# Francesco215/autoregressive_diffusion

Hardware: AMD Instinct MI355X
Metric: denoiser-step frames/sec at 1/2/4/8 MI355X; 64-frame Lunar-Lander seq (higher is better)
Workload: dtype bf16; 1 GPU; Lunar-Lander 64-frame seq, gym EDM2 UNet 46.2M (gym_train.py:37-47), 8 seq/GPU (gym_train.py:55 micro_batch_size), step = EDM2Loss fwd + bwd + grad all-reduce + [grad-norm clip +] AdamW + 2 EMA profiles, 3:1 mix of 3-D/2-D steps; global_batch=8, seq_len=64, parallelism=dp1, hip_graph=False

## Files before the change

### autoregressive_diffusion_amd/_lib.py

```python
import ctypes as C
import os

import torch

_HERE = os.path.dirname(os.path.abspath(__file__))
LIB_PATH = os.path.join(_HERE, os.environ.get("ONIRIS_LIB_NAME", "liboniris_hip.so"))

if not os.path.exists(LIB_PATH):
    raise ImportError(f"{LIB_PATH} not found: build the HIP extension first (make -j8 at the repo root); "
                      "there is no CPU/PyTorch fallback for the denoiser kernels")

lib = C.CDLL(LIB_PATH)

c_void_p, c_int, c_float, c_int32, c_int64, c_size_t = C.c_void_p, C.c_int, C.c_float, C.c_int32, C.c_int64, C.c_size_t


class WeightDesc(C.Structure):
    _fields_ = [("w", c_void_p), ("grad", c_void_p), ("wf", c_void_p), ("wb", c_void_p), ("dwp", c_void_p), ("dws", c_void_p),
                ("cout", c_int32), ("cin", c_int32), ("taps", c_int32), ("kt", c_int32),
                ("CoutP", c_int32), ("CinP", c_int32), ("CoutPb", c_int32), ("CinPb", c_int32),
                ("row_start", c_int32), ("perm3", c_int32), ("gain", c_float), ("nsplit_cap", c_int32),
                ("nsplit", c_void_p), ("tile_start", c_int32), ("pad_", c_int32)]


# ... 42 lines not shown
                ("dout", c_void_p), ("delta", c_void_p), ("dq", c_void_p), ("dk", c_void_p), ("dv", c_void_p),
                ("BH", c_int32), ("Lq", c_int32), ("Lk", c_int32), ("D", c_int32), ("mask_mode", c_int32), ("P", c_int32),
                ("T", c_int32), ("q_frame_off", c_int32), ("scale", c_float), ("pad_", c_int32)]


EPI_NONE, EPI_EMB_SILU, EPI_MPSUM, EPI_ACT_BWD = 0, 1, 2, 3

_SIGS = {
    "oniris_last_error": (C.c_char_p, []),
    "oniris_abi_version": (c_int, []),
    "oniris_struct_sizes": (c_int, [c_void_p]),
    "oniris_profile_arm": (c_int, [c_void_p, c_void_p]),
    "oniris_profile_disarm": (c_int, []),
    "oniris_set_cu_reserve": (c_int, [c_int]),
    "oniris_set_ew_nt_bytes": (c_int64, [c_int64]),
    "oniris_frame_attn_bwd": (c_int, [c_void_p, c_void_p]),
    "oniris_frame_attn_qkv_fwd": (c_int, [c_void_p, c_void_p, c_void_p, c_int64, c_int, c_int, c_void_p]),
    "oniris_frame_attn_qkv_bwd": (c_int, [c_void_p, c_void_p, c_void_p, c_void_p, c_void_p, c_int64, c_int, c_int, c_void_p]),
    "oniris_conv_f32": (c_int, [c_void_p, c_void_p, c_void_p, c_int64, c_int, c_int, c_int, c_int, c_int, c_void_p]),
    "oniris_wgrad_f32": (c_int, [c_void_p, c_void_p, c_void_p, c_int64, c_int, c_int, c_int, c_int, c_int, c_void_p]),
    "oniris_attn_f32_fwd": (c_int, [c_void_p, c_void_p]),
    "oniris_attn_f32_bwd": (c_int, [c_void_p, c_void_p]),
    "oniris_census": (c_int, [c_int]),
    "oniris_census_read": (c_int64, [C.c_char_p, c_int64]),
    "oniris_train_mask": (c_int, [c_int, c_int, c_void_p, c_void_p, C.POINTER(c_int)]),
    "oniris_infer_mask": (c_int, [c_int, c_int, c_void_p, c_void_p, C.POINTER(c_int)]),
    "oniris_mask_transpose": (c_int, [c_int, c_int, c_void_p, c_void_p, c_void_p, c_void_p]),
    "oniris_attn_schedule": (c_int, [c_int, c_int, c_void_p, c_int, c_void_p, c_int]),
    "oniris_weight_prep": (c_int, [c_void_p, c_int, c_int, c_int, c_int, c_void_p]),
    "oniris_weight_bwd": (c_int, [c_void_p, c_int, c_int, c_void_p]),
# ... 202 lines not shown
```

### autoregressive_diffusion_amd/csrc/common.h

```cpp
#pragma once
#include <hip/hip_runtime.h>
#include <hip/hip_ext.h>
#include <stdint.h>
#include <stdio.h>
#include <string.h>

typedef __bf16 bf16;
typedef __attribute__((ext_vector_type(8))) __bf16 bf16x8;
typedef __attribute__((ext_vector_type(4))) __bf16 bf16x4;
typedef __attribute__((ext_vector_type(2))) __bf16 bf16x2;
typedef __attribute__((ext_vector_type(4))) short s16x4;
typedef __attribute__((ext_vector_type(16))) float f32x16;
typedef __attribute__((ext_vector_type(4))) float f32x4;
typedef __attribute__((ext_vector_type(4))) unsigned int u32x4;

#define ONIRIS_OK 0
#define ONIRIS_EINVAL (-1)
#define ONIRIS_ELAUNCH (-2)
#define ONIRIS_EUNSUPPORTED (-3)

void oniris_set_error(const char* fmt, ...);

#define ONIRIS_CHECK_ARG(cond, ...)                \
  do {                                             \
// ... 38 lines not shown
  oniris_launch_tagged(nullptr, kern, grid, block, stream, args...);
}

long long oniris_ew_nt_bytes(void);
template <bool NT, typename V>
__device__ __forceinline__ V ldv(const V* p) {
  if constexpr (NT) return __builtin_nontemporal_load(p);
  else return *p;
}
template <bool NT, typename V>
__device__ __forceinline__ void stv(V* p, V v) {
  if constexpr (NT) __builtin_nontemporal_store(v, p);
  else *p = v;
}

extern int oniris_cu_reserve;
int oniris_persistent_wgs(void);

static inline int cdiv(int a, int b) { return (a + b - 1) / b; }
static inline int roundup(int a, int b) { return cdiv(a, b) * b; }

#ifdef __HIPCC__
__device__ __forceinline__ float bf2f(bf16 v) { return (float)v; }
__device__ __forceinline__ bf16 f2bf(float v) { return (bf16)v; }

__device__ __forceinline__ f32x16 mfma32(bf16x8 a, bf16x8 b, f32x16 c) {
  return __builtin_amdgcn_mfma_f32_32x32x16_bf16(a, b, c, 0, 0, 0);
}
__device__ __forceinline__ float sigmoid_fast(float z) {
  return __builtin_amdgcn_rcpf(1.f + __builtin_amdgcn_exp2f(-1.4426950408889634f * z));
}
__device__ __forceinline__ float act_adjoint_da(float da, float xo) {
  const float sg = sigmoid_fast(xo);
  const float one_m = 1.f - sg;
  const float u = __builtin_fmaf(one_m, xo, 1.f);
  float g = sg * u;
  g = g * da;
  return g * (1.0f / 0.596f);
}
__device__ __forceinline__ float act_adjoint_dxo(float g, float dxo_scale, float dxo) { return __builtin_fmaf(dxo_scale, dxo, g); }
__device__ __forceinline__ float act_adjoint_out(float g, float w, bool has_add, float add) {
  return has_add ? __builtin_fmaf(w, g, add) : g * w;
}
__device__ __forceinline__ int mfma_row(int r, int lane) { return (r & 3) + 8 * (r >> 2) + 4 * (lane >> 5); }

__device__ __forceinline__ float wave_sum(float v) {
#pragma unroll
  for (int o = 32; o > 0; o >>= 1) v += __shfl_xor(v, o);
  return v;
}
__device__ __forceinline__ float wave_max(float v) {
#pragma unroll
  for (int o = 32; o > 0; o >>= 1) v = fmaxf(v, __shfl_xor(v, o));
  return v;
}

__device__ __forceinline__ float block_sum(float v, float* red) {
  v = wave_sum(v);
  const int w = threadIdx.x >> 6, nw = blockDim.x >> 6;
  __syncthreads();
  if ((threadIdx.x & 63) == 0) red[w] = v;
  __syncthreads();
  float t = 0.f;
  for (int i = 0; i < nw; ++i) t += red[i];
  return t;
}
#endif
```

### autoregressive_diffusion_amd/csrc/elementwise.hip

```cpp
#include <cstdlib>
#include "common.h"
#include "../../include/oniris.h"

#define SILU_SCALE (1.0f / 0.596f)

__device__ __forceinline__ float silu_f(float z) { return z * sigmoid_fast(z); }
__device__ __forceinline__ float dsilu_f(float z) {
  const float sg = sigmoid_fast(z);
  return sg * (1.f + z * (1.f - sg));
}

template <bool NORM, bool NT>
__global__ __launch_bounds__(256) void act_fwd_kernel(const bf16* __restrict__ x, const bf16* __restrict__ skip,
                                                      bf16* __restrict__ xo, bf16* __restrict__ a,
                                                      float* __restrict__ sden, long long npix, int C1, int C2, float w1,
                                                      float w2, int rs, int Ho, int Wo) {
  const int C = C1 + C2, G = C >> 3;
  const long long gid = (long long)blockIdx.x * 256 + threadIdx.x;
  const long long pix = gid / G;
  const int cg = (int)(gid % G);
  const bool ok = pix < npix;
  float v[8];
#pragma unroll
  for (int i = 0; i < 8; ++i) v[i] = 0.f;
// ... 148 lines not shown
  const int C = C1 + C2;
  ONIRIS_CHECK_ARG(da && xo && dx && npix > 0 && C1 > 0 && C1 % 8 == 0 && C2 >= 0 && C2 % 8 == 0 && (C2 == 0 || dskip),
                   "act_bwd: bad arguments");
  ONIRIS_CHECK_ARG(!norm || ((C / 8) <= 64 && ((C / 8) & (C / 8 - 1)) == 0 && sden), "act_bwd: pixel norm needs C/8 = 2^k <= 64");
  const long long nthr = npix * (C / 8);
  const dim3 grid((unsigned)((nthr + 255) / 256));
  const bool nt = (long long)npix * C * 2 >= oniris_ew_nt_bytes();
#define ACT_BWD_LAUNCH(NORM_, NT_) ONIRIS_KLAUNCH((act_bwd_kernel<NORM_, NT_>), grid, dim3(256), 0, stream, (const bf16*)da, (const bf16*)dxo, (const bf16*)xo, sden, (bf16*)dx, (bf16*)dskip, (const bf16*)dadd, (long long)npix, C1, C2, w1, w2, dxo_scale)
  if (norm) { if (nt) ACT_BWD_LAUNCH(true, true); else ACT_BWD_LAUNCH(true, false); }
  else { if (nt) ACT_BWD_LAUNCH(false, true); else ACT_BWD_LAUNCH(false, false); }
#undef ACT_BWD_LAUNCH
  ONIRIS_LAUNCH_CHECK();
  return ONIRIS_OK;
}

template <bool NT>
__global__ __launch_bounds__(256) void emb_silu_bwd_kernel(const bf16* __restrict__ du, const bf16* __restrict__ y,
                                                           const float* __restrict__ c, bf16* __restrict__ dy,
                                                           float* __restrict__ dc, int P, int C, int pix_per_block,
                                                           int c_pitch) {
  __shared__ float acc[512];
  const int n = blockIdx.x, G = C >> 3;
  const int cg = threadIdx.x % G, pl = threadIdx.x / G, npl = 256 / G;
  for (int i = threadIdx.x; i < C; i += 256) acc[i] = 0.f;
  __syncthreads();
  float cv[8], part[8];
#pragma unroll
  for (int i = 0; i < 8; ++i) { cv[i] = 0.f; part[i] = 0.f; }
  if (pl < npl) {
    const float4 c0 = *(const float4*)(c + (size_t)n * c_pitch + cg * 8), c1 = *(const float4*)(c + (size_t)n * c_pitch + cg * 8 + 4);
    cv[0] = c0.x; cv[1] = c0.y; cv[2] = c0.z; cv[3] = c0.w; cv[4] = c1.x; cv[5] = c1.y; cv[6] = c1.z; cv[7] = c1.w;
    const int p0 = blockIdx.y * pix_per_block;
    const int p1 = min(P, p0 + pix_per_block);
    for (int p = p0 + pl; p < p1; p += npl) {
      const size_t off = ((size_t)n * P + p) * C + cg * 8;
      const bf16x8 duv = ldv<NT>((const bf16x8*)(du + off)), yv = ldv<NT>((const bf16x8*)(y + off));
      bf16x8 o;
#pragma unroll
      for (int i = 0; i < 8; ++i) {
        const float yy = bf2f(yv[i]);
        const float dz = bf2f(duv[i]) * dsilu_f(yy * cv[i]) * SILU_SCALE;
        o[i] = f2bf(dz * cv[i]);
        part[i] += dz * yy;
      }
      stv<NT>((bf16x8*)(dy + off), o);
    }
  }
  if ((G & (G - 1)) == 0) {
#pragma unroll
    for (int i = 0; i < 8; ++i)
      for (int o = G; o < 64; o <<= 1) part[i] += __shfl_xor(part[i], o);
    for (int q = 0; q < 256 / 64; ++q) {
      if ((int)(threadIdx.x >> 6) == q && (int)(threadIdx.x & 63) < G)
#pragma unroll
        for (int i = 0; i < 8; ++i) acc[cg * 8 + i] += part[i];
      __syncthreads();
    }
  } else {
    for (int q = 0; q < npl; ++q) {
      if (pl == q)
#pragma unroll
        for (int i = 0; i < 8; ++i) acc[cg * 8 + i] += part[i];
      __syncthreads();
    }
  }
  for (int i = threadIdx.x; i < C; i += 256) atomicAdd(dc + (size_t)n * C + i, acc[i]);
}

__global__ void zero_f32_kernel(float* __restrict__ p, size_t n) {
  const size_t i = (size_t)blockIdx.x * blockDim.x + threadIdx.x;
  if (i < n) p[i] = 0.f;
}

extern "C" int oniris_emb_silu_bwd(const void* du, const void* y, const float* c, void* dy, float* dc, int N, int P,
                                   int C, int c_pitch, int dc_is_zero, oniris_stream_t stream_) {
  hipStream_t stream = (hipStream_t)stream_;
  ONIRIS_CHECK_ARG(du && y && c && dy && dc && N > 0 && P > 0 && C > 0 && C % 8 == 0 && C <= 512,
                   "emb_silu_bwd: bad arguments (C %% 8 == 0, C <= 512)");
  int slices = 1;
  const int npl = 256 / (C / 8) > 0 ? 256 / (C / 8) : 1;
  static int tgt = -1;
  if (tgt < 0) { const char* e = getenv("ONIRIS_EMB_SILU_BLOCKS"); tgt = e ? atoi(e) : 1024; }
  while (slices < 2 && P / (slices * 2) >= npl * 4 && (long long)N * slices < tgt) slices *= 2;
  const int ppb = cdiv(P, slices);
  const size_t ndc = (size_t)N * C;
  if (!dc_is_zero) ONIRIS_KLAUNCH(zero_f32_kernel, dim3((unsigned)((ndc + 255) / 256)), dim3(256), 0, stream, dc, ndc);
  const int cp = c_pitch > 0 ? c_pitch : C;
  ONIRIS_CHECK_ARG(cp >= C && cp % 4 == 0, "emb_silu_bwd: c_pitch must be a multiple of 4 and >= C");
  if ((long long)N * P * C * 2 >= oniris_ew_nt_bytes())
    ONIRIS_KLAUNCH(emb_silu_bwd_kernel<true>, dim3(N, slices), dim3(256), 0, stream, (const bf16*)du, (const bf16*)y, c,
                       (bf16*)dy, dc, P, C, ppb, cp);
  else
    ONIRIS_KLAUNCH(emb_silu_bwd_kernel<false>, dim3(N, slices), dim3(256), 0, stream, (const bf16*)du, (const bf16*)y, c,
                       (bf16*)dy, dc, P, C, ppb, cp);
  ONIRIS_LAUNCH_CHECK();
  return ONIRIS_OK;
}

template <bool NT>
__global__ void mpsum_bwd_kernel(const bf16* __restrict__ g, const bf16* __restrict__ out, bf16* __restrict__ dres,
                                 bf16* __restrict__ dv, size_t n8, float ta, float tb, float clip) {
  for (size_t i = (size_t)blockIdx.x * blockDim.x + threadIdx.x; i < n8; i += (size_t)gridDim.x * blockDim.x) {
    const bf16x8 gv = ldv<NT>((const bf16x8*)(g + i * 8));
    bf16x8 a, b;
    if (clip > 0.f) {
      const bf16x8 ov = ldv<NT>((const bf16x8*)(out + i * 8));
#pragma unroll
      for (int k = 0; k < 8; ++k) {
        const float gg = (fabsf(bf2f(ov[k])) < clip) ? bf2f(gv[k]) : 0.f;
// ... 707 lines not shown
```

### autoregressive_diffusion_amd/csrc/misc.cpp

```cpp
#include <cstdlib>
#include <stdarg.h>
#include <stdio.h>
#include <string.h>
#include <algorithm>
#include <map>
#include <mutex>
#include <string>
#include <vector>
#include <cxxabi.h>
#include <dlfcn.h>
#include <hip/hip_runtime.h>
#include "common.h"
#include "../../include/oniris.h"

static thread_local char g_err[512] = "";

void oniris_set_error(const char* fmt, ...) {
  va_list ap;
  va_start(ap, fmt);
  vsnprintf(g_err, sizeof(g_err), fmt, ap);
  va_end(ap);
}

extern "C" const char* oniris_last_error(void) { return g_err; }
// ... 15 lines not shown
static long long g_ew_nt_bytes = -1;
long long oniris_ew_nt_bytes(void) {
  if (g_ew_nt_bytes < 0) {
    const char* e = getenv("ONIRIS_EW_NT_MB");
    const long long mb = e ? atoll(e) : 96;
    g_ew_nt_bytes = mb <= 0 ? (1LL << 62) : mb * (1LL << 20);
  }
  return g_ew_nt_bytes;
}
extern "C" long long oniris_set_ew_nt_bytes(long long bytes) {
  const long long old = oniris_ew_nt_bytes();
  g_ew_nt_bytes = bytes < 0 ? (1LL << 62) : bytes;
  return old;
}

int oniris_census_on = 0;
static std::mutex g_census_mu;
static std::map<std::pair<const void*, std::string>, long long> g_census;
void oniris_census_note(const void* h, const char* tag) {
  std::lock_guard<std::mutex> lock(g_census_mu);
  ++g_census[std::make_pair(h, std::string(tag ? tag : ""))];
}
extern "C" int oniris_census(int on) {
  std::lock_guard<std::mutex> lock(g_census_mu);
  if (on) g_census.clear();
  oniris_census_on = on ? 1 : 0;
  return ONIRIS_OK;
}
static std::string census_name(const void* h) {
  const char* raw = hipKernelNameRefByPtr(h, nullptr);
// ... 164 lines not shown
```

### autoregressive_diffusion_amd/csrc/weights.hip

```cpp
#include <cstdlib>
#include "common.h"
#include "../../include/oniris.h"

#define W_EPS 1e-4f

__device__ __forceinline__ const OnirisWeightDesc* find_desc(const OnirisWeightDesc* d, int n, int row) {
  int lo = 0, hi = n - 1;
  while (lo < hi) {
    int mid = (lo + hi + 1) >> 1;
    if (d[mid].row_start <= row) lo = mid; else hi = mid - 1;
  }
  return d + lo;
}

__device__ __forceinline__ int perm_row(const OnirisWeightDesc* d, int co) {
  if (!d->perm3) return co;
  const int C = d->cout / 3;
  return (co % 3) * C + co / 3;
}

__device__ __forceinline__ const OnirisWeightDesc* find_desc_tile(const OnirisWeightDesc* d, int n, int tile) {
  int lo = 0, hi = n - 1;
  while (lo < hi) {
    int mid = (lo + hi + 1) >> 1;
// ... 324 lines not shown
}

extern "C" int oniris_sqnorm(const float* g, size_t n, float* out, oniris_stream_t stream_) {
  hipStream_t stream = (hipStream_t)stream_;
  ONIRIS_CHECK_ARG(g && out, "sqnorm: null pointer");
  size_t nb = (n / 4 + 255) / 256;
  if (nb > ONIRIS_SQNORM_WS) nb = ONIRIS_SQNORM_WS;
  if (nb == 0) nb = 1;
  ONIRIS_KLAUNCH(sqnorm_partial_kernel, dim3((unsigned)nb), dim3(256), 0, stream, g, n, out + 1);
  ONIRIS_LAUNCH_CHECK();
  ONIRIS_KLAUNCH(sqnorm_final_kernel, dim3(1), dim3(256), 0, stream, (const float*)(out + 1), (int)nb, out);
  ONIRIS_LAUNCH_CHECK();
  return ONIRIS_OK;
}

__global__ __launch_bounds__(256) void gconv_bwd_prep_kernel(const bf16* __restrict__ dout, const bf16* __restrict__ out,
                                                             const bf16* __restrict__ y3, const float* __restrict__ ca,
                                                             const float* __restrict__ cb,
                                                             float* __restrict__ S1, float* __restrict__ S2,
                                                             bf16* __restrict__ dy3, int S, int T, size_t PC) {
  __shared__ float red[16];
  const int bt = blockIdx.x, b = bt / T, t = bt % T;
  const bf16* y3f = y3 + (size_t)bt * PC;
  bf16* dy3f = dy3 + (size_t)bt * PC;
  float s1[2] = {0.f, 0.f}, s2[2] = {0.f, 0.f};
  float c[2];
  const bf16* df[2];
  const bf16* of[2];
  for (int s = 0; s < S; ++s) {
    const size_t n = (size_t)(b * S + s) * T + t;
    c[s] = cb[n]; df[s] = dout + n * PC; of[s] = out + n * PC;
  }
  const size_t per = ((PC / 8 + gridDim.y - 1) / gridDim.y) * 8, e_lo = blockIdx.y * per, e_hi = (e_lo + per < PC) ? e_lo + per : PC;
  for (size_t e = e_lo + (size_t)threadIdx.x * 8; e < e_hi; e += 256 * 8) {
    const bf16x8 yv = *(const bf16x8*)(y3f + e);
    float acc[8];
#pragma unroll
    for (int i = 0; i < 8; ++i) acc[i] = 0.f;
    for (int s = 0; s < S; ++s) {
      const bf16x8 dv = *(const bf16x8*)(df[s] + e);
      const bf16x8 ov = *(const bf16x8*)(of[s] + e);
#pragma unroll
      for (int i = 0; i < 8; ++i) {
        const float dd = bf2f(dv[i]);
        s1[s] += dd * bf2f(ov[i]); s2[s] += dd * bf2f(yv[i]); acc[i] += c[s] * dd;
      }
    }
    bf16x8 o;
#pragma unroll
    for (int i = 0; i < 8; ++i) o[i] = f2bf(acc[i]);
    *(bf16x8*)(dy3f + e) = o;
  }
  for (int s = 0; s < S; ++s) {
    const float a = block_sum(s1[s], red), bsum = block_sum(s2[s], red);
    if (threadIdx.x == 0) { const size_t n = (size_t)(b * S + s) * T + t; atomicAdd(S1 + n, (a - cb[n] * bsum) / ca[n]); atomicAdd(S2 + n, bsum); }
  }
}

template <int MODE, bool NT>
__global__ __launch_bounds__(1024) void gconv_bwd_fused_kernel(const bf16* g, const bf16* __restrict__ raw,
                                                              const bf16* __restrict__ y3, const float* __restrict__ ca,
                                                              const float* __restrict__ cb, const float* __restrict__ cs,
                                                              const bf16* __restrict__ xo, bf16* dout,
                                                              bf16* __restrict__ dres, bf16* __restrict__ dy3,
                                                              float* __restrict__ dca, float* __restrict__ dcb,
                                                              float* __restrict__ dcs, int T, int P, int C, float ta,
                                                              float tb, float clip, int pix_per_block, int cs_pitch,
                                                              const int* __restrict__ clip_flag, float* __restrict__ ca_scaled) {
  const bool alias = MODE == 2 && ca_scaled != nullptr;
  const bool masked = MODE == 2 && clip > 0.f && (!alias || *clip_flag != 0);
  __shared__ float red[16];
  __shared__ float accs[2][512];
  const int bt = blockIdx.x, b = bt / T, t = bt % T;
  const size_t PC = (size_t)P * C;
  const int G8 = C >> 3;
  const int NTH = blockDim.x;
  const int cg = threadIdx.x % G8, pl = threadIdx.x / G8, npl = NTH / G8;
  if (MODE == 1)
    for (int i = threadIdx.x; i < 2 * 512; i += NTH) (&accs[0][0])[i] = 0.f;
  __syncthreads();
  float s1[2] = {0.f, 0.f}, s2[2] = {0.f, 0.f};
  float part[2][8];
#pragma unroll
  for (int s = 0; s < 2; ++s)
#pragma unroll
    for (int i = 0; i < 8; ++i) part[s][i] = 0.f;
  size_t nn[2];
  float cbv[2], cv[2][8];
#pragma unroll
  for (int s = 0; s < 2; ++s) {
    nn[s] = (size_t)(b * 2 + s) * T + t;
    cbv[s] = cb[nn[s]];
#pragma unroll
    for (int i = 0; i < 8; ++i) cv[s][i] = 1.f;
    if (MODE == 1 && pl < npl) {
      const float4 c0 = *(const float4*)(cs + nn[s] * cs_pitch + cg * 8), c1 = *(const float4*)(cs + nn[s] * cs_pitch + cg * 8 + 4);
      cv[s][0] = c0.x; cv[s][1] = c0.y; cv[s][2] = c0.z; cv[s][3] = c0.w;
      cv[s][4] = c1.x; cv[s][5] = c1.y; cv[s][6] = c1.z; cv[s][7] = c1.w;
    }
  }
  if (pl < npl) {
    const int p0 = blockIdx.y * pix_per_block, p1 = min(P, p0 + pix_per_block);
    for (int p = p0 + pl; p < p1; p += npl) {
      const size_t off = (size_t)p * C + cg * 8;
      const bf16x8 yv3 = ldv<NT>((const bf16x8*)(y3 + (size_t)bt * PC + off));
      float acc3[8];
#pragma unroll
      for (int i = 0; i < 8; ++i) acc3[i] = 0.f;
#pragma unroll
      for (int s = 0; s < 2; ++s) {
        const size_t o = nn[s] * PC + off;
        const bf16x8 gv = ldv<NT>((const bf16x8*)(g + o));
        const bf16x8 rv = ldv<NT>((const bf16x8*)(raw + o));
        bf16x8 dv, drv;
        bf16x8 xv;
        if (masked) xv = ldv<NT>((const bf16x8*)(xo + o));
#pragma unroll
        for (int i = 0; i < 8; ++i) {
          const float r_ = bf2f(rv[i]);
          float d;
          if (MODE == 1) {
            const float z = r_ * cv[s][i];
            const float sg = sigmoid_fast(z);
            const float dz = bf2f(gv[i]) * (sg * (1.f + z * (1.f - sg))) * (1.0f / 0.596f);
            part[s][i] += dz * r_;
            d = dz * cv[s][i];
          } else {
            float gg = bf2f(gv[i]);
            if (masked && !(fabsf(bf2f(xv[i])) < clip)) gg = 0.f;
            drv[i] = f2bf(gg * ta);
            d = gg * tb;
            if (alias) dv[i] = f2bf(gg);
          }
          float dr = d;
          if (!alias) { dv[i] = f2bf(d); dr = bf2f(dv[i]); }
          s1[s] += dr * r_; s2[s] += dr * bf2f(yv3[i]); acc3[i] += cbv[s] * dr;
        }
        if (!alias || masked) stv<NT>((bf16x8*)(dout + o), dv);
        if (MODE == 2 && dres) stv<NT>((bf16x8*)(dres + o), drv);
      }
      bf16x8 o3;
#pragma unroll
      for (int i = 0; i < 8; ++i) o3[i] = f2bf(acc3[i]);
      stv<NT>((bf16x8*)(dy3 + (size_t)bt * PC + off), o3);
    }
  }
  if (MODE == 1 && (G8 & (G8 - 1)) == 0) {
#pragma unroll
    for (int s = 0; s < 2; ++s)
#pragma unroll
      for (int i = 0; i < 8; ++i)
        for (int o = G8; o < 64; o <<= 1) part[s][i] += __shfl_xor(part[s][i], o);
    for (int q = 0; q < NTH / 64; ++q) {
      if ((int)(threadIdx.x >> 6) == q && (int)(threadIdx.x & 63) < G8)
#pragma unroll
        for (int s = 0; s < 2; ++s)
#pragma unroll
          for (int i = 0; i < 8; ++i) accs[s][cg * 8 + i] += part[s][i];
      __syncthreads();
    }
// ... 18 lines not shown
  if (MODE == 1) {
    __syncthreads();
    for (int i = threadIdx.x; i < C; i += NTH) {
      atomicAdd(dcs + nn[0] * C + i, accs[0][i]); atomicAdd(dcs + nn[1] * C + i, accs[1][i]);
    }
  }
}

extern "C" int oniris_gconv_bwd_fused(int mode, const void* g, const void* raw, const void* y3, const float* coef_own,
                                      const float* coef_ctx, const float* cscale, const void* xo, void* dout, void* dres,
                                      void* dy3, float* d_coef_own, float* d_coef_ctx, float* d_cscale, int B, int T,
                                      int P, int C, float ta, float tb, float clip, int cscale_pitch,
                                      const int32_t* clip_flag, float* coef_own_scaled, oniris_stream_t stream_) {
  hipStream_t stream = (hipStream_t)stream_;
  ONIRIS_CHECK_ARG((mode == 1 || mode == 2) && g && raw && y3 && coef_own && coef_ctx && dout && dy3 && d_coef_own &&
                   d_coef_ctx && B > 0 && T > 0 && P > 0 && C % 8 == 0 && C <= 512, "gconv_bwd_fused: bad arguments");
  ONIRIS_CHECK_ARG(mode != 1 || (cscale && d_cscale), "gconv_bwd_fused: mode 1 needs cscale / d_cscale");
  ONIRIS_CHECK_ARG(mode != 2 || ((dres || coef_own_scaled) && (clip <= 0.f || xo)),
                   "gconv_bwd_fused: mode 2 needs dres (optional under the aliasing protocol) and xo when clipping");
  ONIRIS_CHECK_ARG((mode == 2 || (!clip_flag && !coef_own_scaled)) && (!clip_flag || coef_own_scaled) &&
                   (!coef_own_scaled || clip <= 0.f || clip_flag),
                   "gconv_bwd_fused: coef_own_scaled selects the aliasing protocol (mode 2); with clip > 0 it needs clip_flag");
  ONIRIS_CHECK_ARG(!coef_own_scaled || dout == g, "gconv_bwd_fused: the aliasing protocol masks g in place (pass dout = g)");
  int slices = 1;
  static int nth1 = -1;
  if (nth1 < 0) { const char* e = getenv("ONIRIS_GCONV_BWD_THREADS"); nth1 = e ? atoi(e) : 256; }
  const int nth = (mode == 1 && (long long)P * (C / 8) >= 4096) ? nth1 : 256;
  const int npl = nth / (C / 8) > 0 ? nth / (C / 8) : 1;
  static int tgt1 = -1;
  if (tgt1 < 0) { const char* e = getenv("ONIRIS_GCONV_BWD_BLOCKS"); tgt1 = e ? atoi(e) : 512; }
  const int tgt = (mode == 1) ? tgt1 : 2048;
  while (slices < 2 && P / (slices * 2) >= npl * 2 && (long long)B * T * slices < tgt) slices *= 2;
  const int ppb = cdiv(P, slices);
  const int csp = cscale_pitch > 0 ? cscale_pitch : C;
  ONIRIS_CHECK_ARG(csp >= C && csp % 4 == 0, "gconv_bwd_fused: cscale_pitch must be a multiple of 4 and >= C");
  const bool nt = 2LL * B * T * P * C * 2 >= oniris_ew_nt_bytes();
#define GCONV_BWD_LAUNCH(MODE_, NT_, NTH_, FLAG_, CAS_) ONIRIS_KLAUNCH((gconv_bwd_fused_kernel<MODE_, NT_>), dim3(B * T, slices), dim3(NTH_), 0, stream, (const bf16*)g, \
                       (const bf16*)raw, (const bf16*)y3, coef_own, coef_ctx, cscale, (const bf16*)xo, (bf16*)dout, \
                       (bf16*)dres, (bf16*)dy3, d_coef_own, d_coef_ctx, d_cscale, T, P, C, ta, tb, clip, ppb, csp, FLAG_, CAS_)
  if (mode == 1) { if (nt) GCONV_BWD_LAUNCH(1, true, nth, nullptr, nullptr); else GCONV_BWD_LAUNCH(1, false, nth, nullptr, nullptr); }
  else { if (nt) GCONV_BWD_LAUNCH(2, true, 256, (const int*)clip_flag, coef_own_scaled); else GCONV_BWD_LAUNCH(2, false, 256, (const int*)clip_flag, coef_own_scaled); }
#undef GCONV_BWD_LAUNCH
  ONIRIS_LAUNCH_CHECK();
  return ONIRIS_OK;
}

extern "C" int oniris_gconv_bwd_prep(const void* dout, const void* out, const void* y3, const float* coef_own,
                                     const float* coef_ctx, float* S1, float* S2, void* dy3, int B, int S, int T,
                                     int64_t frame_elems,
                                     oniris_stream_t stream_) {
  hipStream_t stream = (hipStream_t)stream_;
  ONIRIS_CHECK_ARG(dout && out && y3 && coef_own && coef_ctx && S1 && S2 && dy3 && B > 0 && T > 0 && (S == 1 || S == 2) &&
                   frame_elems > 0 && frame_elems % 8 == 0, "gconv_bwd_prep: bad arguments");
  int slices = 1;
  while (slices < 2 && (long long)B * T * slices < 1024 && frame_elems / (slices * 2) >= 256 * 8 * 2) slices *= 2;
  ONIRIS_KLAUNCH(gconv_bwd_prep_kernel, dim3(B * T, slices), dim3(256), 0, stream, (const bf16*)dout, (const bf16*)out,
                     (const bf16*)y3, coef_own, coef_ctx, S1, S2, (bf16*)dy3, S, T, (size_t)frame_elems);
  ONIRIS_LAUNCH_CHECK();
  return ONIRIS_OK;
}
```

### autoregressive_diffusion_amd/ops.py

```python
import ctypes
import math
import numpy as np
import torch

from . import _lib
from ._lib import lib, check, OnirisError

BF16 = torch.bfloat16


_raw_stream = getattr(torch._C, "_cuda_getCurrentRawStream", None)


def _stream():
    if _raw_stream is not None:
        return ctypes.c_void_p(_raw_stream(torch.cuda.current_device()))
    return ctypes.c_void_p(torch.cuda.current_stream().cuda_stream)


def _p(t):
    return None if t is None else t.data_ptr()


def _need_gpu(*ts):
# ... 81 lines not shown
def set_cu_reserve(k):
    global _cu_reserve
    old = lib.oniris_set_cu_reserve(int(k))
    if old < 0:
        check(old, "set_cu_reserve")
    _cu_reserve = (int(k) + 7) // 8 * 8
    return old


if int(__import__("os").environ.get("ONIRIS_COMM_CUS_ALWAYS", "0")) > 0:
    set_cu_reserve(int(__import__("os").environ["ONIRIS_COMM_CUS_ALWAYS"]))


def set_ew_nt_bytes(nbytes):
    return int(lib.oniris_set_ew_nt_bytes(int(nbytes)))


def census_start():
    check(lib.oniris_census(1), "census")


def census_peek():
    return _census_read()


def census_stop():
    check(lib.oniris_census(0), "census")
    return _census_read()


# ... 2133 lines not shown
```

### include/oniris.h

```cpp
#ifndef ONIRIS_H
#define ONIRIS_H
#include <stddef.h>
#include <stdint.h>

#ifdef __cplusplus
extern "C" {
#endif

typedef void* oniris_stream_t;

const char* oniris_last_error(void);
int oniris_abi_version(void);
int oniris_profile_arm(void* start_event, void* stop_event);
int oniris_profile_disarm(void);
int oniris_set_cu_reserve(int k);
long long oniris_set_ew_nt_bytes(long long bytes);
int oniris_census(int on);
long long oniris_census_read(char* buf , long long cap);
int oniris_struct_sizes(int32_t* out4 );

int oniris_train_mask(int n_frames, int image_size, int32_t* kv_num_blocks, int32_t* kv_indices, int* block_size);
int oniris_infer_mask(int n_frames, int image_size, int32_t* kv_num_blocks, int32_t* kv_indices, int* block_size);
int oniris_mask_transpose(int n_rows, int n_cols, const int32_t* kv_num_blocks, const int32_t* kv_indices,
                          int32_t* q_num_blocks, int32_t* q_indices);

typedef struct OnirisWeightDesc {
  float* w;
  float* grad;
  void* wf;
  void* wb;
  void* dwp;
// ... 359 lines not shown
```

Before: 8796 latent-frames/s.

## Software-pipeline loads in gconv/emb-SiLU backward elementwise kernels with depth-2 prefetch

Adds a generic prepass_loop helper that double-buffers per-thread vector loads (loads D iterations ahead, with scheduling barriers and register pins) and applies it to emb_silu_bwd, gconv_bwd_prep and gconv_bwd_fused. The aim is to hide global-memory latency in these bandwidth-bound backward kernels by keeping more loads in flight per thread. It also switches to 32-bit offset arithmetic with new size guards, uses fma forms, and fixes gconv_bwd_fused at 256 threads, dropping the env-selectable thread count. More live registers could lower occupancy, and the changed FMA order alters rounding slightly. A runtime knob allows falling back to depth 1.

```diff
diff --git a/autoregressive_diffusion_amd/_lib.py b/autoregressive_diffusion_amd/_lib.py
--- a/autoregressive_diffusion_amd/_lib.py
+++ b/autoregressive_diffusion_amd/_lib.py
@@ -80,6 +80,7 @@
     "oniris_profile_disarm": (c_int, []),
     "oniris_set_cu_reserve": (c_int, [c_int]),
     "oniris_set_ew_nt_bytes": (c_int64, [c_int64]),
+    "oniris_set_prepass_depth": (c_int, [c_int]),
     "oniris_frame_attn_bwd": (c_int, [c_void_p, c_void_p]),
     "oniris_frame_attn_qkv_fwd": (c_int, [c_void_p, c_void_p, c_void_p, c_int64, c_int, c_int, c_void_p]),
     "oniris_frame_attn_qkv_bwd": (c_int, [c_void_p, c_void_p, c_void_p, c_void_p, c_void_p, c_int64, c_int, c_int, c_void_p]),
diff --git a/autoregressive_diffusion_amd/csrc/common.h b/autoregressive_diffusion_amd/csrc/common.h
--- a/autoregressive_diffusion_amd/csrc/common.h
+++ b/autoregressive_diffusion_amd/csrc/common.h
@@ -76,6 +76,11 @@
   else *p = v;
 }
 
+#ifndef ONIRIS_PREPASS_DEPTH
+#define ONIRIS_PREPASS_DEPTH 2
+#endif
+int oniris_prepass_depth(void);
+
 extern int oniris_cu_reserve;
 int oniris_persistent_wgs(void);
 
@@ -104,6 +109,10 @@
 __device__ __forceinline__ float act_adjoint_out(float g, float w, bool has_add, float add) {
   return has_add ? __builtin_fmaf(w, g, add) : g * w;
 }
+__device__ __forceinline__ float dsilu_fma(float z) {
+  const float sg = sigmoid_fast(z);
+  return sg * __builtin_fmaf(z, 1.f - sg, 1.f);
+}
 __device__ __forceinline__ int mfma_row(int r, int lane) { return (r & 3) + 8 * (r >> 2) + 4 * (lane >> 5); }
 
 __device__ __forceinline__ float wave_sum(float v) {
@@ -127,4 +136,63 @@
   for (int i = 0; i < nw; ++i) t += red[i];
   return t;
 }
+
+template <typename T>
+__device__ __forceinline__ T* at32(T* base, unsigned off) { return (T*)((const char*)base + (off * (unsigned)sizeof(T))); }
+
+#define PREPASS_FENCE() __builtin_amdgcn_sched_barrier(0)
+__device__ __forceinline__ void prepass_pin(float& v) { asm volatile("" : "+v"(v)); }
+
+template <int D, typename V, typename I, typename L, typename W, typename P>
+__device__ __forceinline__ void prepass_loop(I first, I end, I stride, L&& load, W&& work, P&& pin) {
+  if constexpr (D == 1) {
+    for (I i = first; i < end; i += stride) {
+      V v;
+      load(v, i);
+      work(v, i);
+    }
+  } else {
+    V cur[D], nxt[D];
+    I i = first;
+    if (i + (D - 1) * stride < end) {
+#pragma unroll
+      for (int k = 0; k < D; ++k) load(cur[k], i + k * stride);
+      while (i + (3 * D - 1) * stride < end) {
+#pragma unroll
+        for (int k = 0; k < D; ++k) load(nxt[k], i + (D + k) * stride);
+        PREPASS_FENCE();
+#pragma unroll
+        for (int k = 0; k < D; ++k) { work(cur[k], i + k * stride); pin(); PREPASS_FENCE(); }
+#pragma unroll
+        for (int k = 0; k < D; ++k) load(cur[k], i + (2 * D + k) * stride);
+        PREPASS_FENCE();
+#pragma unroll
+        for (int k = 0; k < D; ++k) { work(nxt[k], i + (D + k) * stride); pin(); PREPASS_FENCE(); }
+        i += 2 * D * stride;
+      }
+      if (i + (2 * D - 1) * stride < end) {
+#pragma unroll
+        for (int k = 0; k < D; ++k) load(nxt[k], i + (D + k) * stride);
+        PREPASS_FENCE();
+#pragma unroll
+        for (int k = 0; k < D; ++k) { work(cur[k], i + k * stride); pin(); PREPASS_FENCE(); }
+#pragma unroll
+        for (int k = 0; k < D; ++k) { work(nxt[k], i + (D + k) * stride); pin(); PREPASS_FENCE(); }
+        i += 2 * D * stride;
+      } else {
+#pragma unroll
+        for (int k = 0; k < D; ++k) { work(cur[k], i + k * stride); pin(); PREPASS_FENCE(); }
+        i += D * stride;
+      }
+    }
+    if (i < end) {
+#pragma unroll
+      for (int k = 0; k < D - 1; ++k)
+        if (i + k * stride < end) load(cur[k], i + k * stride);
+#pragma unroll
+      for (int k = 0; k < D - 1; ++k)
+        if (i + k * stride < end) { work(cur[k], i + k * stride); pin(); }
+    }
+  }
+}
 #endif
diff --git a/autoregressive_diffusion_amd/csrc/elementwise.hip b/autoregressive_diffusion_amd/csrc/elementwise.hip
--- a/autoregressive_diffusion_amd/csrc/elementwise.hip
+++ b/autoregressive_diffusion_amd/csrc/elementwise.hip
@@ -186,7 +186,23 @@
   return ONIRIS_OK;
 }
 
+struct EmbSiluPix { bf16x8 du, y; };
+
 template <bool NT>
+__device__ __forceinline__ void emb_silu_pix(const EmbSiluPix& v, const float (&cv)[8], float (&part)[8], bf16* __restrict__ dy) {
+#pragma clang fp contract(off)
+  bf16x8 o;
+#pragma unroll
+  for (int i = 0; i < 8; ++i) {
+    const float yy = bf2f(v.y[i]);
+    const float dz = bf2f(v.du[i]) * dsilu_fma(yy * cv[i]) * SILU_SCALE;
+    o[i] = f2bf(dz * cv[i]);
+    part[i] = __builtin_fmaf(dz, yy, part[i]);
+  }
+  stv<NT>((bf16x8*)dy, o);
+}
+
+template <bool NT, int D>
 __global__ __launch_bounds__(256) void emb_silu_bwd_kernel(const bf16* __restrict__ du, const bf16* __restrict__ y,
                                                            const float* __restrict__ c, bf16* __restrict__ dy,
                                                            float* __restrict__ dc, int P, int C, int pix_per_block,
@@ -204,19 +220,20 @@
     cv[0] = c0.x; cv[1] = c0.y; cv[2] = c0.z; cv[3] = c0.w; cv[4] = c1.x; cv[5] = c1.y; cv[6] = c1.z; cv[7] = c1.w;
     const int p0 = blockIdx.y * pix_per_block;
     const int p1 = min(P, p0 + pix_per_block);
-    for (int p = p0 + pl; p < p1; p += npl) {
-      const size_t off = ((size_t)n * P + p) * C + cg * 8;
-      const bf16x8 duv = ldv<NT>((const bf16x8*)(du + off)), yv = ldv<NT>((const bf16x8*)(y + off));
-      bf16x8 o;
-#pragma unroll
-      for (int i = 0; i < 8; ++i) {
-        const float yy = bf2f(yv[i]);
-        const float dz = bf2f(duv[i]) * dsilu_f(yy * cv[i]) * SILU_SCALE;
-        o[i] = f2bf(dz * cv[i]);
-        part[i] += dz * yy;
-      }
-      stv<NT>((bf16x8*)(dy + off), o);
-    }
+    const size_t fo = (size_t)n * P * C;
+    const bf16* duf = du + fo;
+    const bf16* yf = y + fo;
+    bf16* dyf = dy + fo;
+    prepass_loop<D, EmbSiluPix>(p0 + pl, p1, npl,
+      [&](EmbSiluPix& v, int p) {
+        const unsigned off = (unsigned)p * C + cg * 8;
+        v.du = ldv<NT>((const bf16x8*)at32(duf, off)); v.y = ldv<NT>((const bf16x8*)at32(yf, off));
+      },
+      [&](const EmbSiluPix& v, int p) { emb_silu_pix<NT>(v, cv, part, at32(dyf, (unsigned)p * C + cg * 8)); },
+      [&]() {
+#pragma unroll
+        for (int i = 0; i < 8; ++i) prepass_pin(part[i]);
+      });
   }
   if ((G & (G - 1)) == 0) {
 #pragma unroll
@@ -247,8 +264,8 @@
 extern "C" int oniris_emb_silu_bwd(const void* du, const void* y, const float* c, void* dy, float* dc, int N, int P,
                                    int C, int c_pitch, int dc_is_zero, oniris_stream_t stream_) {
   hipStream_t stream = (hipStream_t)stream_;
-  ONIRIS_CHECK_ARG(du && y && c && dy && dc && N > 0 && P > 0 && C > 0 && C % 8 == 0 && C <= 512,
-                   "emb_silu_bwd: bad arguments (C %% 8 == 0, C <= 512)");
+  ONIRIS_CHECK_ARG(du && y && c && dy && dc && N > 0 && P > 0 && C > 0 && C % 8 == 0 && C <= 512 && (long long)P * C < (1LL << 31),
+                   "emb_silu_bwd: bad arguments (C %% 8 == 0, C <= 512, P * C < 2^31)");
   int slices = 1;
   const int npl = 256 / (C / 8) > 0 ? 256 / (C / 8) : 1;
   static int tgt = -1;
@@ -259,12 +276,13 @@
   if (!dc_is_zero) ONIRIS_KLAUNCH(zero_f32_kernel, dim3((unsigned)((ndc + 255) / 256)), dim3(256), 0, stream, dc, ndc);
   const int cp = c_pitch > 0 ? c_pitch : C;
   ONIRIS_CHECK_ARG(cp >= C && cp % 4 == 0, "emb_silu_bwd: c_pitch must be a multiple of 4 and >= C");
-  if ((long long)N * P * C * 2 >= oniris_ew_nt_bytes())
-    ONIRIS_KLAUNCH(emb_silu_bwd_kernel<true>, dim3(N, slices), dim3(256), 0, stream, (const bf16*)du, (const bf16*)y, c,
-                       (bf16*)dy, dc, P, C, ppb, cp);
-  else
-    ONIRIS_KLAUNCH(emb_silu_bwd_kernel<false>, dim3(N, slices), dim3(256), 0, stream, (const bf16*)du, (const bf16*)y, c,
-                       (bf16*)dy, dc, P, C, ppb, cp);
+  const bool nt = (long long)N * P * C * 2 >= oniris_ew_nt_bytes();
+  const bool deep = oniris_prepass_depth() != 1;
+#define EMB_SILU_BWD_LAUNCH(NT_, D_) ONIRIS_KLAUNCH((emb_silu_bwd_kernel<NT_, D_>), dim3(N, slices), dim3(256), 0, stream, (const bf16*)du, \
+                       (const bf16*)y, c, (bf16*)dy, dc, P, C, ppb, cp)
+  if (nt) { if (deep) EMB_SILU_BWD_LAUNCH(true, ONIRIS_PREPASS_DEPTH); else EMB_SILU_BWD_LAUNCH(true, 1); }
+  else { if (deep) EMB_SILU_BWD_LAUNCH(false, ONIRIS_PREPASS_DEPTH); else EMB_SILU_BWD_LAUNCH(false, 1); }
+#undef EMB_SILU_BWD_LAUNCH
   ONIRIS_LAUNCH_CHECK();
   return ONIRIS_OK;
 }
diff --git a/autoregressive_diffusion_amd/csrc/misc.cpp b/autoregressive_diffusion_amd/csrc/misc.cpp
--- a/autoregressive_diffusion_amd/csrc/misc.cpp
+++ b/autoregressive_diffusion_amd/csrc/misc.cpp
@@ -53,6 +53,16 @@
   return old;
 }
 
+static int g_prepass_depth = ONIRIS_PREPASS_DEPTH;
+int oniris_prepass_depth(void) { return g_prepass_depth; }
+extern "C" int oniris_set_prepass_depth(int depth) {
+  const int old = g_prepass_depth;
+  if (depth <= 0) depth = ONIRIS_PREPASS_DEPTH;
+  ONIRIS_CHECK_ARG(depth == 1 || depth == ONIRIS_PREPASS_DEPTH, "set_prepass_depth: this build has depth 1 and depth %d", ONIRIS_PREPASS_DEPTH);
+  g_prepass_depth = depth;
+  return old;
+}
+
 int oniris_census_on = 0;
 static std::mutex g_census_mu;
 static std::map<std::pair<const void*, std::string>, long long> g_census;
diff --git a/autoregressive_diffusion_amd/csrc/weights.hip b/autoregressive_diffusion_amd/csrc/weights.hip
--- a/autoregressive_diffusion_amd/csrc/weights.hip
+++ b/autoregressive_diffusion_amd/csrc/weights.hip
@@ -362,6 +362,32 @@
   return ONIRIS_OK;
 }
 
+struct GconvPrepVec { bf16x8 y3, d[2], o[2]; };
+
+__device__ __forceinline__ void gconv_prep_vec(const GconvPrepVec& v, int S, const float (&c)[2], float (&s1)[2], float (&s2)[2],
+                                               bf16* __restrict__ dy3) {
+#pragma clang fp contract(off)
+  float acc[8];
+#pragma unroll
+  for (int i = 0; i < 8; ++i) acc[i] = 0.f;
+#pragma unroll
+  for (int s = 0; s < 2; ++s)
+    if (s < S) {
+#pragma unroll
+      for (int i = 0; i < 8; ++i) {
+        const float dd = bf2f(v.d[s][i]);
+        s1[s] = __builtin_fmaf(dd, bf2f(v.o[s][i]), s1[s]);
+        s2[s] = __builtin_fmaf(dd, bf2f(v.y3[i]), s2[s]);
+        acc[i] = __builtin_fmaf(c[s], dd, acc[i]);
+      }
+    }
+  bf16x8 o;
+#pragma unroll
+  for (int i = 0; i < 8; ++i) o[i] = f2bf(acc[i]);
+  *(bf16x8*)dy3 = o;
+}
+
+template <int D>
 __global__ __launch_bounds__(256) void gconv_bwd_prep_kernel(const bf16* __restrict__ dout, const bf16* __restrict__ out,
                                                              const bf16* __restrict__ y3, const float* __restrict__ ca,
                                                              const float* __restrict__ cb,
@@ -372,49 +398,99 @@
   const bf16* y3f = y3 + (size_t)bt * PC;
   bf16* dy3f = dy3 + (size_t)bt * PC;
   float s1[2] = {0.f, 0.f}, s2[2] = {0.f, 0.f};
-  float c[2];
-  const bf16* df[2];
-  const bf16* of[2];
-  for (int s = 0; s < S; ++s) {
-    const size_t n = (size_t)(b * S + s) * T + t;
-    c[s] = cb[n]; df[s] = dout + n * PC; of[s] = out + n * PC;
-  }
+  float c[2] = {0.f, 0.f};
+  const bf16* df[2] = {nullptr, nullptr};
+  const bf16* of[2] = {nullptr, nullptr};
+#pragma unroll
+  for (int s = 0; s < 2; ++s)
+    if (s < S) {
+      const size_t n = (size_t)(b * S + s) * T + t;
+      c[s] = cb[n]; df[s] = dout + n * PC; of[s] = out + n * PC;
+    }
   const size_t per = ((PC / 8 + gridDim.y - 1) / gridDim.y) * 8, e_lo = blockIdx.y * per, e_hi = (e_lo + per < PC) ? e_lo + per : PC;
-  for (size_t e = e_lo + (size_t)threadIdx.x * 8; e < e_hi; e += 256 * 8) {
-    const bf16x8 yv = *(const bf16x8*)(y3f + e);
-    float acc[8];
-#pragma unroll
-    for (int i = 0; i < 8; ++i) acc[i] = 0.f;
-    for (int s = 0; s < S; ++s) {
-      const bf16x8 dv = *(const bf16x8*)(df[s] + e);
-      const bf16x8 ov = *(const bf16x8*)(of[s] + e);
-#pragma unroll
-      for (int i = 0; i < 8; ++i) {
-        const float dd = bf2f(dv[i]);
-        s1[s] += dd * bf2f(ov[i]); s2[s] += dd * bf2f(yv[i]); acc[i] += c[s] * dd;
-      }
-    }
-    bf16x8 o;
-#pragma unroll
-    for (int i = 0; i < 8; ++i) o[i] = f2bf(acc[i]);
-    *(bf16x8*)(dy3f + e) = o;
-  }
-  for (int s = 0; s < S; ++s) {
+  prepass_loop<D, GconvPrepVec>((unsigned)e_lo + threadIdx.x * 8u, (unsigned)e_hi, 256u * 8u,
+    [&](GconvPrepVec& v, unsigned e) {
+      v.y3 = *(const bf16x8*)at32(y3f, e);
+#pragma unroll
+      for (int s = 0; s < 2; ++s)
+        if (s < S) { v.d[s] = *(const bf16x8*)at32(df[s], e); v.o[s] = *(const bf16x8*)at32(of[s], e); }
+    },
+    [&](const GconvPrepVec& v, unsigned e) { gconv_prep_vec(v, S, c, s1, s2, at32(dy3f, e)); },
+    [&]() { prepass_pin(s1[0]); prepass_pin(s1[1]); prepass_pin(s2[0]); prepass_pin(s2[1]); });
+#pragma unroll
+  for (int s = 0; s < 2; ++s) {
+    if (s >= S) break;
     const float a = block_sum(s1[s], red), bsum = block_sum(s2[s], red);
     if (threadIdx.x == 0) { const size_t n = (size_t)(b * S + s) * T + t; atomicAdd(S1 + n, (a - cb[n] * bsum) / ca[n]); atomicAdd(S2 + n, bsum); }
   }
 }
 
+struct GconvPix { bf16x8 y3, g[2], raw[2], xo[2]; };
+
+struct GconvFrames { const bf16* g[2]; const bf16* raw[2]; const bf16* xo[2]; const bf16* y3; bf16* dout[2]; bf16* dres[2]; bf16* dy3; };
+
 template <int MODE, bool NT>
-__global__ __launch_bounds__(1024) void gconv_bwd_fused_kernel(const bf16* g, const bf16* __restrict__ raw,
-                                                              const bf16* __restrict__ y3, const float* __restrict__ ca,
-                                                              const float* __restrict__ cb, const float* __restrict__ cs,
-                                                              const bf16* __restrict__ xo, bf16* dout,
-                                                              bf16* __restrict__ dres, bf16* __restrict__ dy3,
-                                                              float* __restrict__ dca, float* __restrict__ dcb,
-                                                              float* __restrict__ dcs, int T, int P, int C, float ta,
-                                                              float tb, float clip, int pix_per_block, int cs_pitch,
-                                                              const int* __restrict__ clip_flag, float* __restrict__ ca_scaled) {
+__device__ __forceinline__ void gconv_pix_load(GconvPix& v, const GconvFrames& f, unsigned off, bool masked) {
+  v.y3 = ldv<NT>((const bf16x8*)at32(f.y3, off));
+#pragma unroll
+  for (int s = 0; s < 2; ++s) {
+    v.g[s] = ldv<NT>((const bf16x8*)at32(f.g[s], off));
+    v.raw[s] = ldv<NT>((const bf16x8*)at32(f.raw[s], off));
+    if (masked) v.xo[s] = ldv<NT>((const bf16x8*)at32(f.xo[s], off));
+  }
+}
+
+template <int MODE, bool NT>
+__device__ __forceinline__ void gconv_pix_work(const GconvPix& v, const GconvFrames& f, unsigned off, const float (&cv)[2][8],
+                                               const float (&cbv)[2], float ta, float tb, float clip, bool alias, bool masked,
+                                               float (&s1)[2], float (&s2)[2], float (&part)[2][8]) {
+#pragma clang fp contract(off)
+  float acc3[8];
+#pragma unroll
+  for (int i = 0; i < 8; ++i) acc3[i] = 0.f;
+#pragma unroll
+  for (int s = 0; s < 2; ++s) {
+    bf16x8 dv, drv;
+#pragma unroll
+    for (int i = 0; i < 8; ++i) {
+      const float r_ = bf2f(v.raw[s][i]);
+      float d;
+      if (MODE == 1) {
+        const float dz = bf2f(v.g[s][i]) * dsilu_fma(r_ * cv[s][i]) * (1.0f / 0.596f);
+        part[s][i] = __builtin_fmaf(dz, r_, part[s][i]);
+        d = dz * cv[s][i];
+      } else {
+        float gg = bf2f(v.g[s][i]);
+        if (masked && !(fabsf(bf2f(v.xo[s][i])) < clip)) gg = 0.f;
+        drv[i] = f2bf(gg * ta);
+        d = gg * tb;
+        if (alias) dv[i] = f2bf(gg);
+      }
+      float dr = d;
+      if (!alias) { dv[i] = f2bf(d); dr = bf2f(dv[i]); }
+      if (MODE == 1) { s1[s] += dr * r_; s2[s] += dr * bf2f(v.y3[i]); }
+      else { s1[s] = __builtin_fmaf(dr, r_, s1[s]); s2[s] = __builtin_fmaf(dr, bf2f(v.y3[i]), s2[s]); }
+      acc3[i] = __builtin_fmaf(cbv[s], dr, acc3[i]);
+    }
+    if (!alias || masked) stv<NT>((bf16x8*)at32(f.dout[s], off), dv);
+    if (MODE == 2 && f.dres[s]) stv<NT>((bf16x8*)at32(f.dres[s], off), drv);
+  }
+  bf16x8 o3;
+#pragma unroll
+  for (int i = 0; i < 8; ++i) o3[i] = f2bf(acc3[i]);
+  stv<NT>((bf16x8*)at32(f.dy3, off), o3);
+}
+
+template <int MODE, bool NT, int D>
+__global__ __launch_bounds__(256) void gconv_bwd_fused_kernel(const bf16* g, const bf16* __restrict__ raw,
+                                                             const bf16* __restrict__ y3, const float* __restrict__ ca,
+                                                             const float* __restrict__ cb, const float* __restrict__ cs,
+                                                             const bf16* __restrict__ xo, bf16* dout,
+                                                             bf16* __restrict__ dres, bf16* __restrict__ dy3,
+                                                             float* __restrict__ dca, float* __restrict__ dcb,
+                                                             float* __restrict__ dcs, int T, int P, int C, float ta,
+                                                             float tb, float clip, int pix_per_block, int cs_pitch,
+                                                             const int* __restrict__ clip_flag, float* __restrict__ ca_scaled) {
   const bool alias = MODE == 2 && ca_scaled != nullptr;
   const bool masked = MODE == 2 && clip > 0.f && (!alias || *clip_flag != 0);
   __shared__ float red[16];
@@ -422,7 +498,7 @@
   const int bt = blockIdx.x, b = bt / T, t = bt % T;
   const size_t PC = (size_t)P * C;
   const int G8 = C >> 3;
-  const int NTH = blockDim.x;
+  const int NTH = 256;
   const int cg = threadIdx.x % G8, pl = threadIdx.x / G8, npl = NTH / G8;
   if (MODE == 1)
     for (int i = threadIdx.x; i < 2 * 512; i += NTH) (&accs[0][0])[i] = 0.f;
@@ -449,49 +525,27 @@
   }
   if (pl < npl) {
     const int p0 = blockIdx.y * pix_per_block, p1 = min(P, p0 + pix_per_block);
-    for (int p = p0 + pl; p < p1; p += npl) {
-      const size_t off = (size_t)p * C + cg * 8;
-      const bf16x8 yv3 = ldv<NT>((const bf16x8*)(y3 + (size_t)bt * PC + off));
-      float acc3[8];
-#pragma unroll
-      for (int i = 0; i < 8; ++i) acc3[i] = 0.f;
-#pragma unroll
-      for (int s = 0; s < 2; ++s) {
-        const size_t o = nn[s] * PC + off;
-        const bf16x8 gv = ldv<NT>((const bf16x8*)(g + o));
-        const bf16x8 rv = ldv<NT>((const bf16x8*)(raw + o));
-        bf16x8 dv, drv;
-        bf16x8 xv;
-        if (masked) xv = ldv<NT>((const bf16x8*)(xo + o));
-#pragma unroll
-        for (int i = 0; i < 8; ++i) {
-          const float r_ = bf2f(rv[i]);
-          float d;
-          if (MODE == 1) {
-            const float z = r_ * cv[s][i];
-            const float sg = sigmoid_fast(z);
-            const float dz = bf2f(gv[i]) * (sg * (1.f + z * (1.f - sg))) * (1.0f / 0.596f);
-            part[s][i] += dz * r_;
-            d = dz * cv[s][i];
-          } else {
-            float gg = bf2f(gv[i]);
-            if (masked && !(fabsf(bf2f(xv[i])) < clip)) gg = 0.f;
-            drv[i] = f2bf(gg * ta);
-            d = gg * tb;
-            if (alias) dv[i] = f2bf(gg);
-          }
-          float dr = d;
-          if (!alias) { dv[i] = f2bf(d); dr = bf2f(dv[i]); }
-          s1[s] += dr * r_; s2[s] += dr * bf2f(yv3[i]); acc3[i] += cbv[s] * dr;
+    GconvFrames f;
+#pragma unroll
+    for (int s = 0; s < 2; ++s) {
+      f.g[s] = g + nn[s] * PC; f.raw[s] = raw + nn[s] * PC; f.xo[s] = xo ? xo + nn[s] * PC : nullptr;
+      f.dout[s] = dout + nn[s] * PC; f.dres[s] = dres ? dres + nn[s] * PC : nullptr;
+    }
+    f.y3 = y3 + (size_t)bt * PC; f.dy3 = dy3 + (size_t)bt * PC;
+    prepass_loop<D, GconvPix>(p0 + pl, p1, npl,
+      [&](GconvPix& v, int p) { gconv_pix_load<MODE, NT>(v, f, (unsigned)p * C + cg * 8, masked); },
+      [&](const GconvPix& v, int p) {
+        gconv_pix_work<MODE, NT>(v, f, (unsigned)p * C + cg * 8, cv, cbv, ta, tb, clip, alias, masked, s1, s2, part);
+      },
+      [&]() {
+        prepass_pin(s1[0]); prepass_pin(s1[1]); prepass_pin(s2[0]); prepass_pin(s2[1]);
+        if (MODE == 1) {
+#pragma unroll
+          for (int s = 0; s < 2; ++s)
+#pragma unroll
+            for (int i = 0; i < 8; ++i) prepass_pin(part[s][i]);
         }
-        if (!alias || masked) stv<NT>((bf16x8*)(dout + o), dv);
-        if (MODE == 2 && dres) stv<NT>((bf16x8*)(dres + o), drv);
-      }
-      bf16x8 o3;
-#pragma unroll
-      for (int i = 0; i < 8; ++i) o3[i] = f2bf(acc3[i]);
-      stv<NT>((bf16x8*)(dy3 + (size_t)bt * PC + off), o3);
-    }
+      });
   }
   if (MODE == 1 && (G8 & (G8 - 1)) == 0) {
 #pragma unroll
@@ -540,7 +594,8 @@
                                       const int32_t* clip_flag, float* coef_own_scaled, oniris_stream_t stream_) {
   hipStream_t stream = (hipStream_t)stream_;
   ONIRIS_CHECK_ARG((mode == 1 || mode == 2) && g && raw && y3 && coef_own && coef_ctx && dout && dy3 && d_coef_own &&
-                   d_coef_ctx && B > 0 && T > 0 && P > 0 && C % 8 == 0 && C <= 512, "gconv_bwd_fused: bad arguments");
+                   d_coef_ctx && B > 0 && T > 0 && P > 0 && C % 8 == 0 && C <= 512 && (long long)P * C < (1LL << 31),
+                   "gconv_bwd_fused: bad arguments");
   ONIRIS_CHECK_ARG(mode != 1 || (cscale && d_cscale), "gconv_bwd_fused: mode 1 needs cscale / d_cscale");
   ONIRIS_CHECK_ARG(mode != 2 || ((dres || coef_own_scaled) && (clip <= 0.f || xo)),
                    "gconv_bwd_fused: mode 2 needs dres (optional under the aliasing protocol) and xo when clipping");
@@ -549,10 +604,7 @@
                    "gconv_bwd_fused: coef_own_scaled selects the aliasing protocol (mode 2); with clip > 0 it needs clip_flag");
   ONIRIS_CHECK_ARG(!coef_own_scaled || dout == g, "gconv_bwd_fused: the aliasing protocol masks g in place (pass dout = g)");
   int slices = 1;
-  static int nth1 = -1;
-  if (nth1 < 0) { const char* e = getenv("ONIRIS_GCONV_BWD_THREADS"); nth1 = e ? atoi(e) : 256; }
-  const int nth = (mode == 1 && (long long)P * (C / 8) >= 4096) ? nth1 : 256;
-  const int npl = nth / (C / 8) > 0 ? nth / (C / 8) : 1;
+  const int npl = 256 / (C / 8) > 0 ? 256 / (C / 8) : 1;
   static int tgt1 = -1;
   if (tgt1 < 0) { const char* e = getenv("ONIRIS_GCONV_BWD_BLOCKS"); tgt1 = e ? atoi(e) : 512; }
   const int tgt = (mode == 1) ? tgt1 : 2048;
@@ -561,11 +613,14 @@
   const int csp = cscale_pitch > 0 ? cscale_pitch : C;
   ONIRIS_CHECK_ARG(csp >= C && csp % 4 == 0, "gconv_bwd_fused: cscale_pitch must be a multiple of 4 and >= C");
   const bool nt = 2LL * B * T * P * C * 2 >= oniris_ew_nt_bytes();
-#define GCONV_BWD_LAUNCH(MODE_, NT_, NTH_, FLAG_, CAS_) ONIRIS_KLAUNCH((gconv_bwd_fused_kernel<MODE_, NT_>), dim3(B * T, slices), dim3(NTH_), 0, stream, (const bf16*)g, \
+  const bool deep = oniris_prepass_depth() != 1;
+#define GCONV_BWD_LAUNCH(MODE_, NT_, D_, FLAG_, CAS_) ONIRIS_KLAUNCH((gconv_bwd_fused_kernel<MODE_, NT_, D_>), dim3(B * T, slices), dim3(256), 0, stream, (const bf16*)g, \
                        (const bf16*)raw, (const bf16*)y3, coef_own, coef_ctx, cscale, (const bf16*)xo, (bf16*)dout, \
                        (bf16*)dres, (bf16*)dy3, d_coef_own, d_coef_ctx, d_cscale, T, P, C, ta, tb, clip, ppb, csp, FLAG_, CAS_)
-  if (mode == 1) { if (nt) GCONV_BWD_LAUNCH(1, true, nth, nullptr, nullptr); else GCONV_BWD_LAUNCH(1, false, nth, nullptr, nullptr); }
-  else { if (nt) GCONV_BWD_LAUNCH(2, true, 256, (const int*)clip_flag, coef_own_scaled); else GCONV_BWD_LAUNCH(2, false, 256, (const int*)clip_flag, coef_own_scaled); }
+#define GCONV_BWD_DEPTH(MODE_, NT_, FLAG_, CAS_) do { if (deep) GCONV_BWD_LAUNCH(MODE_, NT_, ONIRIS_PREPASS_DEPTH, FLAG_, CAS_); else GCONV_BWD_LAUNCH(MODE_, NT_, 1, FLAG_, CAS_); } while (0)
+  if (mode == 1) { if (nt) GCONV_BWD_DEPTH(1, true, nullptr, nullptr); else GCONV_BWD_DEPTH(1, false, nullptr, nullptr); }
+  else { if (nt) GCONV_BWD_DEPTH(2, true, (const int*)clip_flag, coef_own_scaled); else GCONV_BWD_DEPTH(2, false, (const int*)clip_flag, coef_own_scaled); }
+#undef GCONV_BWD_DEPTH
 #undef GCONV_BWD_LAUNCH
   ONIRIS_LAUNCH_CHECK();
   return ONIRIS_OK;
@@ -577,11 +632,13 @@
                                      oniris_stream_t stream_) {
   hipStream_t stream = (hipStream_t)stream_;
   ONIRIS_CHECK_ARG(dout && out && y3 && coef_own && coef_ctx && S1 && S2 && dy3 && B > 0 && T > 0 && (S == 1 || S == 2) &&
-                   frame_elems > 0 && frame_elems % 8 == 0, "gconv_bwd_prep: bad arguments");
+                   frame_elems > 0 && frame_elems % 8 == 0 && frame_elems < (1LL << 31) - 16 * 2048, "gconv_bwd_prep: bad arguments");
   int slices = 1;
   while (slices < 2 && (long long)B * T * slices < 1024 && frame_elems / (slices * 2) >= 256 * 8 * 2) slices *= 2;
-  ONIRIS_KLAUNCH(gconv_bwd_prep_kernel, dim3(B * T, slices), dim3(256), 0, stream, (const bf16*)dout, (const bf16*)out,
-                     (const bf16*)y3, coef_own, coef_ctx, S1, S2, (bf16*)dy3, S, T, (size_t)frame_elems);
+#define GCONV_PREP_LAUNCH(D_) ONIRIS_KLAUNCH(gconv_bwd_prep_kernel<D_>, dim3(B * T, slices), dim3(256), 0, stream, (const bf16*)dout, \
+                     (const bf16*)out, (const bf16*)y3, coef_own, coef_ctx, S1, S2, (bf16*)dy3, S, T, (size_t)frame_elems)
+  if (oniris_prepass_depth() != 1) GCONV_PREP_LAUNCH(ONIRIS_PREPASS_DEPTH); else GCONV_PREP_LAUNCH(1);
+#undef GCONV_PREP_LAUNCH
   ONIRIS_LAUNCH_CHECK();
   return ONIRIS_OK;
 }
diff --git a/autoregressive_diffusion_amd/ops.py b/autoregressive_diffusion_amd/ops.py
--- a/autoregressive_diffusion_amd/ops.py
+++ b/autoregressive_diffusion_amd/ops.py
@@ -119,6 +119,12 @@
 
 def set_ew_nt_bytes(nbytes):
     return int(lib.oniris_set_ew_nt_bytes(int(nbytes)))
+
+
+def set_prepass_depth(depth):
+    old = int(lib.oniris_set_prepass_depth(int(depth)))
+    check(min(old, 0), "set_prepass_depth")
+    return old
 
 
 def census_start():
diff --git a/include/oniris.h b/include/oniris.h
--- a/include/oniris.h
+++ b/include/oniris.h
@@ -15,6 +15,7 @@
 int oniris_profile_disarm(void);
 int oniris_set_cu_reserve(int k);
 long long oniris_set_ew_nt_bytes(long long bytes);
+int oniris_set_prepass_depth(int depth);
 int oniris_census(int on);
 long long oniris_census_read(char* buf , long long cap);
 int oniris_struct_sizes(int32_t* out4 );
```

Result: no change. 8878 latent-frames/s, median of 6 (+0.9%).
